# edwindn/rl-agent-for-qubit-array-tuning

Measured on AMD Instinct MI355X. Metric: env steps/sec (batched 8-dot 64x64 CSD solves), higher is better.
Workload: dtype f64; 1 GPU; 8-dot array, 4096 parallel envs per GPU, 64x64 CSD, deterministic physics (latching/noise off), 50-step episodes, staggered phases: 820 episode resets (new device + first observation) inside the timed region, synthetic CNN outputs; n_dots=8, envs_per_gpu=4096, resolution=64

## Files before the change

### __graft_entry__.py

```python
import os
import subprocess
import sys

ROOT = os.path.dirname(os.path.abspath(__file__))
PKG = os.path.join(ROOT, "rl-agent-for-qubit-array-tuning_amd")
for _p in (PKG, os.path.join(ROOT, "oracle"), os.path.join(ROOT, "tests")):
    if _p not in sys.path:
        sys.path.insert(0, _p)


def build() -> None:
    csrc = os.path.join(PKG, "csrc")
    subprocess.check_call(["make", "-C", csrc, "libqdsim.so"])
    subprocess.check_call(["make", "-C", os.path.join(ROOT, "tests", "hosttest"), "libqdsim_hosttest.so", "qd_scratch_asan"])
    subprocess.check_call(["make", "-C", os.path.join(ROOT, "tests", "hosttest_wave"), "libqdsim_hosttest_wave.so"])
    subprocess.check_call(["make", "-C", os.path.join(ROOT, "tests", "hosttest_gs"), "libqdsim_hosttest_gs.so"])
    subprocess.check_call(["make", "-C", os.path.join(ROOT, "tests", "hosttest_points"), "libqdsim_hosttest_points.so"])
    subprocess.check_call(["make", "-C", os.path.join(ROOT, "tests", "hosttest_latch"), "libqdsim_hosttest_latch.so"])
    subprocess.check_call(["make", "-C", os.path.join(ROOT, "tests", "gputest_eig"), "libqdsim_gputest_eig.so"])
    subprocess.check_call(["make", "-C", os.path.join(ROOT, "oracle"), "libqdoracle.so"])
    import qadapt_hip
    from qadapt_hip import _lib
    L = _lib.lib()
    missing = [n for n in _lib.EXPORTS if not hasattr(L, n)]
    if missing:
        raise RuntimeError(f"libqdsim.so lacks symbols: {missing}")


def smoke() -> None:
    import numpy as np
    import torch
    import qd_oracle as O
    import helpers as H
    from qadapt_hip.vec_env import VecQuantumDeviceEnv, SyntheticCapacitanceModel

    assert torch.cuda.is_available(), "smoke() needs the MI355X"
    N, R, B, seed = 4, 16, 2, 2024
    env = VecQuantumDeviceEnv(B, num_dots=N, resolution=R, seed=seed, validate=True,
                              capacitance_model=SyntheticCapacitanceModel(3))
    rng = np.random.default_rng(0)
    C = N - 1
    v0 = rng.normal(0, 0.1, (B, C, 3)).astype(np.float32); l0 = rng.uniform(-6, -2, (B, C, 3)).astype(np.float32)
    obs = env.reset(cnn_outputs=(torch.as_tensor(v0).cuda(), torch.as_tensor(l0).cuda()))
    act = rng.uniform(-1, 1, (B, 2 * N - 1)).astype(np.float32)
    v1 = rng.normal(0, 0.1, (B, C, 3)).astype(np.float32); l1 = rng.uniform(-6, -2, (B, C, 3)).astype(np.float32)
    obs, rew, term, trunc = env.step(torch.as_tensor(act).cuda(),
                                     cnn_outputs=(torch.as_tensor(v1).cuda(), torch.as_tensor(l1).cuda()))
    img = obs["image"].cpu().numpy()
    raw, _ = env.raw()
    for e in range(B):
        oe = O.OracleEnv(N, R)
        oe.reset(O.sample_episode(np.random.default_rng(seed + e), N), v0[e], l0[e])
        oobs, (gr, br), _, _ = oe.step(act[e, :N], act[e, N:], v1[e], l1[e])
        r = rew[e].cpu().numpy()
        assert np.allclose(r[:N], gr, rtol=1e-9) and np.allclose(r[N:], br, rtol=1e-9), "reward mismatch"
        H.image_parity(oe, img[e], raw[e])
    env.close()
    print("smoke ok: 4-dot 16x16 batched step matches the oracle")


if __name__ == "__main__":
    build()
    if len(sys.argv) > 1 and sys.argv[1] == "smoke":
        smoke()
```

### include/qdsim.h

```cpp
#ifndef QDSIM_H
#define QDSIM_H

#include <stdint.h>

#ifdef __cplusplus
extern "C" {
#endif

#define QD_OK 0
#define QD_ERR_ARG 1
#define QD_ERR_HIP 2
#define QD_ERR_STATE 3
#define QD_ERR_NOMEM 4

#define QD_FLAG_VALIDATE 1
#define QD_FLAG_PIXEL_SEARCH 2
#define QD_FLAG_RETIRED_TILE_FUSED 4

#define QD_NOISE_SENSOR 1
#define QD_NOISE_RADIAL 2
#define QD_NOISE_LATCH 4

typedef struct qd_handle qd_handle;

typedef struct qd_config {
    int32_t struct_size;
    int32_t n_dot;
    int32_t resolution;
    int32_t batch;
    int32_t max_steps;
    int32_t env_chunk;
    int32_t flags;
    int32_t noise_flags;
    double gate_ramp_start;
    double gate_quadratic_start;
    double barrier_ramp_start;
    double kalman_prior_mean;
    double kalman_prior_variance;
    double kalman_prior_mean_nnn;
    double kalman_variance_threshold;
    double kalman_process_noise;
    uint64_t rng_seed;
    int64_t env_id_offset;
    int32_t use_deltas;
    int32_t sparse_reward;
    int32_t gate_curve_type;
    int32_t update_method;
    int32_t cnn_outputs;
    int32_t num_charge_states;
    double delta_max;
    double gate_curve_exponent;
    double plunger_radius;
    double outer_plunger_radius;
    double outer_plunger_reward_max;
    double barrier_radius;
} qd_config;

#define QD_ALL_CHARGE_STATES(m) (-(m))

#define QD_CURVE_CONSTANT 0
#define QD_CURVE_POLYNOMIAL 1
#define QD_CURVE_EXPONENTIAL 2
#define QD_CURVE_LINEAR 3
#define QD_UPDATE_KALMAN 0
#define QD_UPDATE_DIRECT 1

int qd_param_block_doubles(int n_dot);
int qd_state_block_doubles(int n_dot);
int qd_layout_query(int n_dot, int32_t* out31);

// ... 75 lines not shown
```

### rl-agent-for-qubit-array-tuning_amd/csrc/qd_api.hip

```cpp
#include <hip/hip_runtime.h>
#include <stdio.h>
#include <stdlib.h>
#include <string.h>
#include <new>

#include "qdsim.h"
#include "qd_kernels.h"
#include "qd_fullspace.h"
#include "qd_probe.h"
#include "qd_latch.h"
#include "qd_points.h"
#include "qd_scratch.h"

struct QdStream : QdNoCopy {
    hipStream_t s = nullptr;
    ~QdStream() { if (s) (void)hipStreamDestroy(s); }
    hipError_t create() { return hipStreamCreateWithFlags(&s, hipStreamNonBlocking); }
};
struct QdEvent : QdNoCopy {
    hipEvent_t e = nullptr;
    ~QdEvent() { if (e) (void)hipEventDestroy(e); }
    hipError_t create(unsigned flags = hipEventDisableTiming) { return hipEventCreateWithFlags(&e, flags); }
};

// ... 409 lines not shown
    nz.env_off = b.env_off;
    nz.ser_lo = (uint32_t)b.serial; nz.ser_hi = (uint32_t)(b.serial >> 32);
    nz.tel = b.tel; nz.tel_words = b.tel_words;
    return nz;
}

enum {
    QD_ST_TILE = 1, QD_ST_REDO = 2, QD_ST_STRUCTURE = 4, QD_ST_SOLVE = 8, QD_ST_SELECT = 16,
    QD_ST_SEARCH = QD_ST_TILE | QD_ST_REDO,
    QD_ST_GROUND = QD_ST_STRUCTURE | QD_ST_SOLVE | QD_ST_SELECT,
    QD_ST_ALL = QD_ST_SEARCH | QD_ST_GROUND
};

static int qd_stages(const qd_handle* h) {
    return h->full_m ? QD_ST_GROUND : (h->tile_search ? QD_ST_ALL : QD_ST_ALL & ~QD_ST_TILE);
}

template <int BIN>
static hipError_t qd_launch_solve(const qd_handle* h, const QdLane& ln, hipStream_t s) {
    const dim3 grid((unsigned)h->solve_grid[BIN]);
    QD_DISPATCH_BOOL(qd_validate(h), VAL,
                     qd_k_gs_solve<BIN, VAL><<<grid, dim3(256), 0, s>>>(ln.slabs.p, ln.gtiles.p, ln.gtiles.p + 16, h->gs_batches, h->tstats.p));
    return hipGetLastError();
}

static int qd_launch_ground(const qd_handle* h, const QdEnvBufs& b, const QdLane& ln, const int32_t* env_ids, int base, int cnt,
                            hipStream_t s, int st) {
    const int nb = (h->P + h->ppb - 1) / h->ppb;
    unsigned* tilelist = ln.gtiles.p + 16;
    const bool val = qd_validate(h);
    QdWide wide = h->wide; wide.buf = ln.wide.p;
    const int rec0 = val ? base : 0;
    for (int off = 0; off < cnt; off += h->gs_chunk) {
        const int n = cnt - off < h->gs_chunk ? cnt - off : h->gs_chunk;
        const QdGsGeom g{n, h->C, h->P, nb};
        const unsigned batches = (unsigned)((size_t)n * h->C * nb);
        if (st & QD_ST_STRUCTURE) {
            QD_HIP(hipMemsetAsync(ln.gtiles.p, 0, sizeof(unsigned) * 16, s));
            if (h->full_m) {
#define QD_DISPATCH_FULL(...)                                                                                  \
                if (!wide.capw && h->full_spl == 2) { constexpr int SPL = 2; constexpr bool WIDE = false; __VA_ARGS__; }  \
                else if (h->full_spl == 2) { constexpr int SPL = 2; constexpr bool WIDE = true; __VA_ARGS__; }            \
                else if (h->full_spl == 4) { constexpr int SPL = 4; constexpr bool WIDE = true; __VA_ARGS__; }            \
                else { constexpr int SPL = 8; constexpr bool WIDE = true; __VA_ARGS__; }
                QD_DISPATCH_BOOL(val, VAL, QD_DISPATCH_FULL(QD_DISPATCH_N(h->N,
                    qd_k_full_structure<NN, VAL, SPL, WIDE><<<dim3(batches), dim3(64 * QdFullWpb<SPL>::v), 0, s>>>(env_ids, base + off,
                        rec0 + off, g, h->ppb, h->R, b.params, b.state, b.noise_flags, h->ftab.p, ln.recs.p, ln.slabs.p, ln.gtiles.p, tilelist,
                        h->gs_batches, wide))));
#undef QD_DISPATCH_FULL
            } else {
                QD_DISPATCH_BOOL(val, VAL, QD_DISPATCH_BOOL(batches < (unsigned)h->cus, SMALL, QD_DISPATCH_N(h->N,
                    qd_k_gs_structure<NN, VAL, (SMALL ? 16 : 4)><<<dim3(batches), dim3(64 * (SMALL ? 16 : 4)), 0, s>>>(env_ids, base + off,
                        rec0 + off, g, h->R, b.params, ln.recs.p, b.state, b.noise_flags, ln.slabs.p, ln.gtiles.p, tilelist, h->gs_batches,
                        h->kept))));
            }
            QD_HIP(hipGetLastError());
        }
        if (st & QD_ST_SOLVE) {
            int max_bin = h->N == 2 ? qd_gs_bin(4) : (h->N == 3 ? qd_gs_bin(12) : QD_GS_NBIN - 1);
            if (h->full_m) {
                int M = 0, maxsec = 0;
                qd_full_sizes(h->N, h->full_m, M, maxsec);
                max_bin = qd_gs_bin(maxsec < QD_K ? maxsec : QD_K);
            } else if (h->kept < 2) max_bin = -1;
            else if (qd_gs_bin(h->kept) < max_bin) max_bin = qd_gs_bin(h->kept);
            const bool forked = max_bin >= 9;
            hipStream_t s9 = forked ? ln.side.s : s, s48 = forked ? ln.side2.s : s;
            if (forked) {
                QD_HIP(hipEventRecord(ln.ev_fork.e, s));
                QD_HIP(hipStreamWaitEvent(ln.side.s, ln.ev_fork.e, 0));
                QD_HIP(hipStreamWaitEvent(ln.side2.s, ln.ev_fork.e, 0));
            }
            if (wide.capw) {
                const size_t slots = (size_t)batches * wide.capw, full = (size_t)h->cus * 4;
                const dim3 wgrid((unsigned)(slots < full ? slots : full));
                QD_DISPATCH_BOOL(val, VAL, qd_k_full_solve_wide<VAL><<<wgrid, dim3(64), 0, s>>>(ln.slabs.p, wide, batches, h->tstats.p));
                QD_HIP(hipGetLastError());
            }
            if (max_bin >= 9) QD_HIP(qd_launch_solve<9>(h, ln, s9));
            if (forked) QD_HIP(hipEventRecord(ln.ev_join.e, ln.side.s));
            if (max_bin >= 8) QD_HIP(qd_launch_solve<8>(h, ln, s48));
            if (max_bin >= 7) QD_HIP(qd_launch_solve<7>(h, ln, s48));
            if (max_bin >= 6) QD_HIP(qd_launch_solve<6>(h, ln, s48));
            if (max_bin >= 5) QD_HIP(qd_launch_solve<5>(h, ln, s48));
            if (max_bin >= 4) QD_HIP(qd_launch_solve<4>(h, ln, s48));
            if (forked) QD_HIP(hipEventRecord(ln.ev_join2.e, ln.side2.s));
            if (max_bin >= 0) QD_HIP(qd_launch_solve<0>(h, ln, s));
            if (max_bin >= 1) QD_HIP(qd_launch_solve<1>(h, ln, s));
            if (max_bin >= 2) QD_HIP(qd_launch_solve<2>(h, ln, s));
            if (max_bin >= 3) QD_HIP(qd_launch_solve<3>(h, ln, s));
            if (forked) {
                QD_HIP(hipStreamWaitEvent(s, ln.ev_join.e, 0));
                QD_HIP(hipStreamWaitEvent(s, ln.ev_join2.e, 0));
            }
        }
        if (st & QD_ST_SELECT) {
            if (h->full_m) {
                const unsigned blk = (unsigned)((h->ppb + 63) / 64 * 64);
                QD_DISPATCH_BOOL(val, VAL, QD_DISPATCH_BOOL(wide.capw != 0, WIDE, QD_DISPATCH_N(h->N,
                    qd_k_full_select<NN, VAL, WIDE><<<dim3(batches), dim3(blk), 0, s>>>(env_ids, base + off, rec0 + off, g, h->ppb,
                        b.params, ln.recs.p, b.zraw, b.occ, b.state, b.noise_flags, b.eig, h->ftab.p, ln.slabs.p, wide))));
            } else {
                QD_DISPATCH_BOOL(val, VAL, QD_DISPATCH_N(h->N, QD_DISPATCH_KC(h->kc,
                    qd_k_gs_select<NN, VAL, KK><<<dim3(batches), dim3(QD_GS_BLOCK), 0, s>>>(env_ids, base + off, rec0 + off, g, h->R,
                        b.params, ln.recs.p, b.zraw, b.occ, b.state, b.noise_flags, b.eig, ln.slabs.p))));
            }
            QD_HIP(hipGetLastError());
// ... 547 lines not shown
```

### rl-agent-for-qubit-array-tuning_amd/csrc/qd_groundstate.h

```cpp
#pragma once
#include "qd_pixel.h"
#include "qd_eig.h"

#define QD_GS_PPB 256
#define QD_GS_NBIN 10
QD_HD constexpr int qd_gs_bin(int s) { return s <= 8 ? s - 2 : (s <= 10 ? 7 : (s <= 12 ? 8 : 9)); }
QD_HD constexpr int qd_gs_bin_min(int bin) { return bin <= 6 ? bin + 2 : (bin == 7 ? 9 : (bin == 8 ? 11 : 13)); }

QD_HD unsigned qd_gs_hop(unsigned ci, unsigned cj, unsigned tcq) {
#if defined(__HIP_DEVICE_COMPILE__)
    unsigned ay;
    asm("v_sad_u32 %0, %1, %2, 0" : "=v"(ay) : "v"(ci), "v"(cj));
#else
    const unsigned ay = ci > cj ? ci - cj : cj - ci;
#endif
    const int tz = __builtin_ctz(ay | 0x80000000u);
    const unsigned x = ay + (0xFFFFFFF1u << tz);
    const unsigned t = (tcq >> tz) & 1u;
    return t > x ? t - x : 0u;
}

#if defined(__HIPCC__)

#ifndef QD_NBREG
#define QD_NBREG 6
#endif
#define QD_GS_BLOCK 256
#define QD_LINK_NONE 0xFFFFFFFFu
#define QD_LINK_SINGLE 0xFFFFFFFEu

typedef __attribute__((address_space(3))) double qd_lds_double;
typedef volatile qd_lds_double* qd_lds_vptr;
typedef const volatile qd_lds_double* qd_lds_cvptr;

template <int N>
struct QdWaveLds {
    static constexpr int NS = (2 * (N - 1) - QD_NBREG) > 1 ? (2 * (N - 1) - QD_NBREG) : 1;
    double coef[NS][64];
    unsigned char nidx[NS][64];
    double buf[64];
    double pv[2][16];
    short pfl[2][8];
};
struct QdBlockLds {
    unsigned pool_top;
    unsigned cnt[QD_GS_NBIN];
};

struct QdSlab {
    double* pool; unsigned* link; unsigned char* rank; unsigned* lists; double* aux; unsigned* cnt; double* lam;
};
constexpr int QD_GS_CAP_TAB[QD_GS_NBIN + 1] = {16, 10, 8, 6, 5, 4, 4, 3, 2, 2, 2};
constexpr int QD_GS_OFF_TAB[QD_GS_NBIN + 1] = {0, 16, 26, 34, 40, 45, 49, 53, 56, 58, 60};
constexpr unsigned long long qd_gs_pack_tab(const int* tab, int n, int bits) {
    unsigned long long w = 0;
    for (int b = 0; b < n; ++b) w |= (unsigned long long)tab[b] << (bits * b);
    return w;
}
constexpr unsigned long long QD_GS_CAP_WORD = qd_gs_pack_tab(QD_GS_CAP_TAB, QD_GS_NBIN + 1, 5);
constexpr unsigned long long QD_GS_OFF_WORD = qd_gs_pack_tab(QD_GS_OFF_TAB, QD_GS_NBIN, 6);
QD_HD constexpr int qd_gs_list_cap(int bin) { return QD_GS_PPB * (int)((QD_GS_CAP_WORD >> (5 * bin)) & 31u); }
QD_HD constexpr int qd_gs_list_off(int bin) {
    return QD_GS_PPB * (bin >= QD_GS_NBIN ? QD_GS_OFF_TAB[QD_GS_NBIN] : (int)((QD_GS_OFF_WORD >> (6 * bin)) & 63u));
}
constexpr bool qd_gs_lists_match_definition() {
    int o = 0;
    for (int b = 0; b <= QD_GS_NBIN; ++b) {
        if (qd_gs_list_off(b) != o || qd_gs_list_cap(b) != QD_GS_PPB * (32 / qd_gs_bin_min(b))) return false;
        o += QD_GS_PPB * (32 / qd_gs_bin_min(b));
    }
    return true;
}
static_assert(qd_gs_lists_match_definition(), "QD_GS_CAP_TAB / QD_GS_OFF_TAB: capacity 32 / qd_gs_bin_min(b) per pixel, offsets their running sum");
__host__ __device__ inline int qd_gs_task_doubles(int s, bool validate) {
    const int ne = s * (s + 1) / 2;
    const int n = 2 + ne + (s > QD_EIG_REG ? 4 * s + (validate ? ne : 0) : 0);
    return (n + 1) & ~1;
}
__host__ __device__ inline size_t qd_gs_pool_doubles(bool validate) { return (size_t)QD_GS_PPB * (size_t)qd_gs_task_doubles(32, validate); }
__host__ __device__ inline size_t qd_gs_slab_bytes(bool validate) {
    size_t b = qd_gs_pool_doubles(validate) * 8;
    b += (size_t)QD_GS_PPB * 32 * 4;
    b += (size_t)qd_gs_list_off(QD_GS_NBIN) * 4;
    b += (size_t)QD_GS_PPB * 16;
    b += (size_t)QD_GS_PPB * 32;
    b += 64;
    b += (size_t)qd_gs_list_off(QD_GS_NBIN) * 8;
    return (b + 255) & ~(size_t)255;
}
__host__ __device__ inline QdSlab qd_gs_slab(unsigned char* base, bool validate) {
    QdSlab s;
    s.pool = (double*)base; base += qd_gs_pool_doubles(validate) * 8;
    s.link = (unsigned*)base; base += (size_t)QD_GS_PPB * 32 * 4;
    s.lists = (unsigned*)base; base += (size_t)qd_gs_list_off(QD_GS_NBIN) * 4;
    s.aux = (double*)base; base += (size_t)QD_GS_PPB * 16;
    s.rank = base; base += (size_t)QD_GS_PPB * 32;
    s.cnt = (unsigned*)base; base += 64;
    s.lam = (double*)base;
    return s;
}
__host__ __device__ inline size_t qd_gs_tile_cap(int bin, size_t batches) { return batches * (size_t)((qd_gs_list_cap(bin) + 63) / 64); }
__host__ __device__ inline size_t qd_gs_tile_off(int bin, size_t batches) { size_t o = 0; for (int b = 0; b < bin; ++b) o += qd_gs_tile_cap(b, batches); return o; }

__device__ __forceinline__ unsigned qd_half_ballot(bool p) {
    unsigned long long b = __ballot(p);
    return (unsigned)(b >> (threadIdx.x & 32));
}
__device__ __forceinline__ double qd_half_min(double v) {
#pragma unroll
    for (int o = 16; o > 0; o >>= 1) v = fmin(v, __shfl_xor(v, o, 32));
    return v;
}
__device__ __forceinline__ int qd_wave_max_int(int v) {
#pragma unroll
    for (int o = 32; o > 0; o >>= 1) v = max(v, __shfl_xor(v, o, 64));
    return __builtin_amdgcn_readfirstlane(v);
}

#ifndef QD_GS_ROT_SWIZZLE
#define QD_GS_ROT_SWIZZLE 1
#endif
template <int J, bool UP>
__device__ __forceinline__ unsigned qd_half_rot(unsigned v) {
#if QD_GS_ROT_SWIZZLE
    return (unsigned)__builtin_amdgcn_ds_swizzle((int)v, 0xC000 | ((UP ? 0 : 1) << 10) | (J << 5));
#else
    return (unsigned)__shfl((int)v, ((int)(threadIdx.x & 31) + (UP ? J : 32 - J)) & 31, 32);
#endif
}
template <int J>
__device__ __forceinline__ void qd_gs_hop_rounds(unsigned ecode, unsigned tcq, unsigned& acc) {
    const unsigned hop = qd_gs_hop(ecode, qd_half_rot<J, true>(ecode), tcq);
    acc |= hop << J;
    if constexpr (J < 16) {
        acc |= qd_half_rot<J, false>(hop) << (32 - J);
        qd_gs_hop_rounds<J + 1>(ecode, tcq, acc);
    }
}

template <int N, bool VALIDATE>
__device__ __forceinline__ void qd_ground_structure(const QdPixelRec* __restrict__ rec, bool live, int ps, QdWaveLds<N>& W,
                                                    QdBlockLds& S, const QdSlab& sl, int kept) {
    const int lane = threadIdx.x & 63;
    const int m = lane & 31;
    const int hb = lane & 32;
    const unsigned lt = (1u << m) - 1u;
    qd_lds_vptr buf = (qd_lds_vptr)W.buf;

    const int hh = hb >> 5;
    if (m >= 9 && m < 9 + N - 1) W.pv[hh][m] = rec->tc[m - 9];
    if (m >= 16 && m < 16 + N) W.pfl[hh][m - 16] = (short)rec->fl[m - 16];
    __builtin_amdgcn_wave_barrier();
    const double* pvv = W.pv[hh];
    const bool inK = m < kept;
    const int nvalid = min(rec->nvalid, kept);
    const bool valid = m < nvalid;
    const unsigned code = valid ? (unsigned)rec->idx[m] : 0u;
    unsigned ecode = code;
    ecode = (ecode | (ecode << 8)) & 0x00FF00FFu;
    ecode = (ecode | (ecode << 4)) & 0x0F0F0F0Fu;
    ecode = (ecode | (ecode << 2)) & 0x33333333u;
    const double Fabs = inK ? rec->E[m] : INFINITY;
    const double fshift = qd_half_min(Fabs);
    const double F = Fabs - fshift;

    unsigned tcnz = 0;
#pragma unroll
    for (int d = 0; d < N - 1; ++d) tcnz |= (pvv[9 + d] != 0.0 ? 1u : 0u) << d;
    unsigned tcq = 0;
#pragma unroll
    for (int q = 0; q < N - 1; ++q) tcq |= ((tcnz >> (N - 2 - q)) & 1u) << (4 * q);
    unsigned acc = 0;
    qd_gs_hop_rounds<1>(ecode, tcq, acc);
    unsigned nbrmask = __builtin_rotateleft32(acc, (unsigned)m);
    nbrmask = (valid && live) ? (nbrmask & (nvalid >= 32 ? 0xFFFFFFFFu : ((1u << nvalid) - 1u))) : 0u;
#if defined(QD_ABLATE) && QD_ABLATE == 4
    nbrmask = 0;
#endif
    const int cnt = __popc(nbrmask);
    const int maxcnt = qd_wave_max_int(cnt);
    double radius = 0.0;
    double creg[QD_NBREG]; int jreg[QD_NBREG];
#pragma unroll
    for (int i = 0; i < QD_NBREG; ++i) { creg[i] = 0.0; jreg[i] = m; }
    {
        unsigned rem = nbrmask;
        for (int s = 0; s < maxcnt; ++s) {
            const bool has = rem != 0;
            const int j = has ? __builtin_ctz(rem) : m;
            rem &= rem - 1;
            const unsigned cj = __shfl(ecode, j, 32);
            double c = 0.0;
            if (has) {
                const int Y = (int)cj - (int)ecode;
                const unsigned ay = (unsigned)(Y < 0 ? -Y : Y);
                const int q = __builtin_ctz(ay) >> 2;
                const int d = N - 2 - q;
                const int nd = (int)W.pfl[hh][d] + (int)((ecode >> (4 * (q + 1))) & 3u) - 1;
                const int nd1 = (int)W.pfl[hh][d + 1] + (int)((ecode >> (4 * q)) & 3u) - 1;
                const double t = pvv[9 + d];
                const double prod = (double)((Y < 0) ? nd * (nd1 + 1) : nd1 * (nd + 1));
                double sq_ = 0.0;
                if (prod > 0.0) sq_ = qd_sqrt1(prod);
                c = -t * sq_;
            }
            if (s < QD_NBREG) {
#pragma unroll
                for (int i = 0; i < QD_NBREG; ++i) if (i == s) { creg[i] = c; jreg[i] = j; }
            } else { W.coef[s - QD_NBREG][lane] = c; W.nidx[s - QD_NBREG][lane] = (unsigned char)j; }
            radius += fabs(c);
        }
    }

    unsigned seg = (1u << m) | nbrmask;
    for (int guard = 0; guard < 32; ++guard) {
        unsigned nw = seg, rem = nbrmask;
        for (int s = 0; s < maxcnt; ++s) {
            const bool has = rem != 0;
            const int j = has ? __builtin_ctz(rem) : m;
            rem &= rem - 1;
            nw |= __shfl(seg, j, 32);
        }
        const bool changed = nw != seg;
        seg = nw;
        if (!__any(changed)) break;
    }
    const int ssz = __popc(seg);
    const int r = __popc(seg & lt);
    const int smax = qd_wave_max_int(ssz);

    double comp_lower;
    {
        buf[lane] = F - radius;
        __builtin_amdgcn_wave_barrier();
        double acc = INFINITY;
        unsigned mm = seg;
        for (int it = 0; it < smax; ++it) {
            if (mm) { const int b = __builtin_ctz(mm); mm &= mm - 1; acc = fmin(acc, buf[hb + b]); }
        }
        __builtin_amdgcn_wave_barrier();
        comp_lower = acc;
    }
    const bool active = live && comp_lower <= 0.0;
#if defined(QD_ABLATE) && QD_ABLATE == 3
    const bool solve = false;
#else
    const bool solve = active && ssz > 1;
#endif

    unsigned base = 0, gi = 0;
    if (solve && r == 0) {
        base = atomicAdd(&S.pool_top, (unsigned)qd_gs_task_doubles(ssz, VALIDATE));
        const int bin = qd_gs_bin(ssz);
        gi = (unsigned)qd_gs_list_off(bin) + atomicAdd(&S.cnt[bin], 1u);
        sl.lists[gi] = base;
        if (ssz > 8) sl.pool[base + 1] = (double)ssz;
    }
    base = (unsigned)__shfl((int)base, __builtin_ctz(seg), 32);
    gi = (unsigned)__shfl((int)gi, __builtin_ctz(seg), 32);
    if (live) {
        sl.link[ps * 32 + m] = solve ? gi : (active ? QD_LINK_SINGLE : QD_LINK_NONE);
        sl.rank[ps * 32 + m] = (unsigned char)r;
        if (VALIDATE) {
            const double hn = -qd_half_min(inK ? -(fabs(Fabs) + radius) : INFINITY);
            if (m == 0) { sl.aux[ps] = hn; sl.aux[QD_GS_PPB + ps] = fshift; }
        }
    }
    {
        double* row = sl.pool + base + 2 + (r * (r + 1)) / 2;
        unsigned nrm = 0;
        for (int s = 0; s < maxcnt; ++s) {
            if (s < cnt && solve) {
                int j = jreg[0]; double c = creg[0];
                if (s >= QD_NBREG) { j = (int)W.nidx[s - QD_NBREG][lane]; c = W.coef[s - QD_NBREG][lane]; }
#pragma unroll
                for (int i = 1; i < QD_NBREG; ++i) if (i == s) { j = jreg[i]; c = creg[i]; }
                const int rj = __popc(seg & ((1u << j) - 1u));
                if (rj < r) { row[rj] = c; nrm |= 1u << rj; }
            }
        }
        for (int c = 0; c < smax - 1; ++c)
            if (solve && c < r && !((nrm >> c) & 1u)) row[c] = 0.0;
        if (solve) row[r] = F;
    }
}

template <int S, bool PADDED, bool VALIDATE>
__device__ __forceinline__ int qd_eig_task(double* rec, double& lam) {
    double resid, x[S];
    int its = 0;
    const int sz = PADDED ? (int)rec[1] : S;
    qd_eig_lowest<S, VALIDATE>(rec + 2, lam, x, resid, VALIDATE ? &its : nullptr, sz);
    if (VALIDATE) rec[1] = resid;
    if (sz == S) {
        double2* X2 = reinterpret_cast<double2*>(rec + 2);
#pragma unroll
        for (int i = 0; i + 1 < S; i += 2) X2[i >> 1] = make_double2(x[i], x[i + 1]);
        if (S & 1) rec[2 + S - 1] = x[S - 1];
    } else {
#pragma unroll
        for (int i = 0; i < S; ++i) if (i < sz) rec[2 + i] = x[i];
    }
    return its;
}
template <bool VALIDATE>
__device__ __forceinline__ int qd_eig_task_mem(double* rec, double& lam) {
    const int s = (int)rec[1];
    const int ne = s * (s + 1) / 2;
    double* M = rec + 2;
    double* work = M + ne;
    double* copy = VALIDATE ? work + 4 * s : nullptr;
    if (VALIDATE) for (int e = 0; e < ne; ++e) copy[e] = M[e];
    double resid;
    int its = 0;
    qd_eig_lowest_mem(s, M, work, copy, lam, resid, VALIDATE ? &its : nullptr);
    if (VALIDATE) rec[1] = resid;
    for (int i = 0; i < s; ++i) M[i] = work[3 * s + i];
    return its;
}

template <int N, bool VALIDATE, int KC>
__device__ __forceinline__ void qd_ground_select(const QdPixelRec* __restrict__ rec, int ps, const QdSlab& sl,
                                                 double* occ, double& lam_out, double& resid_out) {
    const unsigned* __restrict__ link = sl.link + ps * 32;
    const unsigned char* __restrict__ rank = sl.rank + ps * 32;
    const double* __restrict__ pool = sl.pool;
    const double* __restrict__ lamd = sl.lam;
    const int nvalid = rec->nvalid;
    unsigned lk[KC];
    double lam[KC];
    {
        const uint4* l4 = reinterpret_cast<const uint4*>(link);
#pragma unroll
        for (int q = 0; q < KC / 4; ++q) { const uint4 v = l4[q]; lk[4 * q] = v.x; lk[4 * q + 1] = v.y; lk[4 * q + 2] = v.z; lk[4 * q + 3] = v.w; }
// ... 64 lines not shown
```

### rl-agent-for-qubit-array-tuning_amd/csrc/qd_kernels.h

```cpp
#pragma once
#include "qd_groundstate.h"
#include "qd_rng.h"

#if defined(__HIPCC__)

struct QdRewardCfg {
    double gate_ramp_start, gate_quadratic_start, barrier_ramp_start;
    int max_steps;
    int use_deltas, sparse, curve;
    double delta_max, curve_exponent;
    double plunger_radius, outer_plunger_radius, outer_plunger_reward_max, barrier_radius;
};

__device__ __forceinline__ double qd_gate_reward(double dist, const QdRewardCfg& rc) {
    if (rc.sparse) {
        if (dist <= rc.plunger_radius) return 1.0;
        if (dist <= rc.outer_plunger_radius) {
            const double nd = (dist - rc.plunger_radius) / (rc.outer_plunger_radius - rc.plunger_radius);
            return rc.outer_plunger_reward_max * (1.0 - nd);
        }
        return 0.0;
    }
    double r;
    if (dist >= rc.gate_ramp_start) r = 0.0;
// ... 163 lines not shown
    if (nv < KC) {
        double dd[N];
#pragma unroll
        for (int i = 0; i < N; ++i) dd[i] = 0.0 - vd[i];
#pragma unroll 1
        for (int i = 0; i < N; ++i) {
            const double t = qd_dotN<N>(spar + L.cdd_inv + i * G, dd);
            double di = dd[0];
#pragma unroll
            for (int j = 1; j < N; ++j) di = (j == i) ? dd[j] : di;
            F0 = fma(di, t, F0);
        }
    }
#pragma unroll
    for (int m = 0; m < KC; ++m) rec->E[m] = (m < nv ? se[m * QD_CAND_BLOCK + threadIdx.x] : F0) * isa;
#pragma unroll
    for (int i = 0; i < N; ++i) rec->fl[i] = fl[i];
    rec->nvalid = nv;
}

struct QdGsGeom { int n_env, C, P, nb; };
__device__ __forceinline__ void qd_gs_locate(const QdGsGeom& g, int batch, int& slot, int& ch, int& p0) {
    slot = batch / (g.C * g.nb);
    const int rem = batch - slot * g.C * g.nb;
    ch = rem / g.nb; p0 = (rem - ch * g.nb) * QD_GS_PPB;
}

__device__ __forceinline__ void qd_gs_publish_tiles(const QdBlockLds& sB, const QdSlab& sl, int batch, unsigned* __restrict__ gtiles,
                                                    unsigned* __restrict__ tilelist, size_t batches_cap) {
    if (threadIdx.x < QD_GS_NBIN) {
        const int bin = threadIdx.x;
        const unsigned nt = sB.cnt[bin];
        sl.cnt[bin] = nt;
        const unsigned ntile = (nt + 63u) >> 6;
        if (ntile) {
            const unsigned start = atomicAdd(&gtiles[bin], ntile);
            unsigned* tl = tilelist + qd_gs_tile_off(bin, batches_cap) + start;
            for (unsigned t = 0; t < ntile; ++t) {
                const unsigned here = nt - t * 64u < 64u ? nt - t * 64u : 64u;
                tl[t] = ((unsigned)batch << 12) | (t << 6) | (here - 1u);
            }
        }
    }
}

#ifndef QD_GS_WAVES
#define QD_GS_WAVES 7
#endif
template <int N, bool VALIDATE, int WPB>
__global__ void __launch_bounds__(64 * WPB, WPB == 4 ? QD_GS_WAVES : 4)
qd_k_gs_structure(const int* __restrict__ env_ids, int env_base, int rec_slot0, QdGsGeom g, int R, const double* __restrict__ params,
                  const QdPixelRec* __restrict__ recs, const double* __restrict__ state, int noise_flags,
                  unsigned char* __restrict__ slabs, unsigned* __restrict__ gtiles, unsigned* __restrict__ tilelist, size_t batches_cap,
                  int kept) {
    const QdLayout L = qd_layout(N);
    __shared__ QdWaveLds<N> sW[WPB];
    __shared__ QdBlockLds sB;
    constexpr int PPW = QD_GS_PPB / WPB;
    const int batch = blockIdx.x;
    const QdSlab sl = qd_gs_slab(slabs + (size_t)batch * qd_gs_slab_bytes(VALIDATE), VALIDATE);
    const int wave = threadIdx.x >> 6, lane = threadIdx.x & 63;
    int slot, ch, p0;
    qd_gs_locate(g, batch, slot, ch, p0);
    const int e = env_ids ? env_ids[env_base + slot] : env_base + slot;
    const double* par = params + (size_t)e * L.size;
    const double* st = state + (size_t)e * L.s_size;
    if (qd_radial_replaced(par, st, L, ch, noise_flags)) {
        if (threadIdx.x < QD_GS_NBIN) sl.cnt[threadIdx.x] = 0;
        return;
    }
    const QdPixelRec* rbase = recs + ((size_t)(rec_slot0 + slot) * g.C + ch) * g.P;
    if (threadIdx.x <= QD_GS_NBIN) { if (threadIdx.x == 0) sB.pool_top = 0; else sB.cnt[threadIdx.x - 1] = 0; }
    __syncthreads();
    QdWaveLds<N>& W = sW[wave];
    for (int it = 0; it < PPW / 2; ++it) {
        const int ps = wave * PPW + it * 2 + (lane >> 5);
        if (p0 + wave * PPW + it * 2 >= g.P) break;
        const int p = p0 + ps;
        const int pc = p < g.P ? p : g.P - 1;
        qd_ground_structure<N, VALIDATE>(rbase + pc, p < g.P, ps, W, sB, sl, kept);
    }
    __syncthreads();
    qd_gs_publish_tiles(sB, sl, batch, gtiles, tilelist, batches_cap);
}

template <int BIN, bool VALIDATE>
__device__ __forceinline__ int qd_gs_solve_task(double* rec, double& lam) {
    if constexpr (BIN <= 6) return qd_eig_task<BIN + 2, false, VALIDATE>(rec, lam);
    else if constexpr (BIN == 7) return qd_eig_task<10, true, VALIDATE>(rec, lam);
    else if constexpr (BIN == 8) return qd_eig_task<12, true, VALIDATE>(rec, lam);
    else return qd_eig_task_mem<VALIDATE>(rec, lam);
}
template <int BIN> struct QdGsSolveWaves { static constexpr int v = BIN <= 1 ? 6 : (BIN == 2 ? 4 : (BIN == 3 ? 3 : (BIN <= 6 ? 2 : (BIN == 9 ? 4 : 1)))); };

template <int BIN, bool VALIDATE>
__global__ void __launch_bounds__(256, QdGsSolveWaves<BIN>::v)
qd_k_gs_solve(unsigned char* __restrict__ slabs, const unsigned* __restrict__ gtiles, const unsigned* __restrict__ tilelist,
              size_t batches_cap, unsigned long long* __restrict__ stats) {
    const int lane = threadIdx.x & 63;
    const unsigned ntile = gtiles[BIN];
    const unsigned* tl = tilelist + qd_gs_tile_off(BIN, batches_cap);
    const unsigned nwaves = gridDim.x * 4u;
    unsigned gt = blockIdx.x * 4u + (threadIdx.x >> 6);
    const size_t slab_bytes = qd_gs_slab_bytes(VALIDATE);
    auto offset_of = [&](unsigned d) -> unsigned {
        const QdSlab sl = qd_gs_slab(slabs + (size_t)(d >> 12) * slab_bytes, VALIDATE);
        return lane <= (int)(d & 63u) ? sl.lists[qd_gs_list_off(BIN) + (int)((d >> 6) & 63u) * 64 + lane] : 0u;
    };
    unsigned desc = gt < ntile ? tl[gt] : 0u;
    unsigned desc1 = gt + nwaves < ntile ? tl[gt + nwaves] : 0u;
    unsigned off = gt < ntile ? offset_of(desc) : 0u;
    for (; gt < ntile; gt += nwaves) {
        const unsigned desc2 = gt + 2u * nwaves < ntile ? tl[gt + 2u * nwaves] : 0u;
        const unsigned off1 = gt + nwaves < ntile ? offset_of(desc1) : 0u;
        const unsigned batch = desc >> 12;
        const int here = (int)(desc & 63u) + 1;
        const QdSlab sl = qd_gs_slab(slabs + (size_t)batch * slab_bytes, VALIDATE);
        int its = 0;
        if (lane < here) {
            double lam;
            its = qd_gs_solve_task<BIN, VALIDATE>(sl.pool + off, lam);
            sl.lam[qd_gs_list_off(BIN) + (int)((desc >> 6) & 63u) * 64 + lane] = lam;
        }
        desc = desc1; desc1 = desc2; off = off1;
        if (VALIDATE && stats) {
            int sum = its, mx = its;
#pragma unroll
            for (int o = 32; o > 0; o >>= 1) { sum += __shfl_xor(sum, o, 64); mx = max(mx, __shfl_xor(mx, o, 64)); }
            if (lane == 0) {
                atomicAdd(&stats[16], (unsigned long long)here); atomicAdd(&stats[17], (unsigned long long)sum);
                atomicAdd(&stats[18], 1ull); atomicAdd(&stats[19], (unsigned long long)mx);
                atomicAdd(&stats[20 + BIN], (unsigned long long)here);
            }
// ... 579 lines not shown
```

### rl-agent-for-qubit-array-tuning_amd/qadapt_hip/_lib.py

```python
from __future__ import annotations

import ctypes
import os
import subprocess

_HERE = os.path.dirname(os.path.abspath(__file__))
CSRC = os.path.join(os.path.dirname(_HERE), "csrc")
LIB_PATH = os.environ.get("QDSIM_LIB", os.path.join(CSRC, "libqdsim.so"))

QD_FLAG_VALIDATE = 1
QD_FLAG_PIXEL_SEARCH = 2
QD_NOISE_SENSOR = 1
QD_NOISE_RADIAL = 2
QD_NOISE_LATCH = 4
QD_MAP_GLOBAL, QD_MAP_PER_SCAN = 0, 1
QD_POINTS_SLOTS = 64
QD_ERR_ARG, QD_ERR_HIP, QD_ERR_STATE = 1, 2, 3

EXPORTS = [
    "qd_param_block_doubles", "qd_state_block_doubles", "qd_layout_query", "qd_create", "qd_destroy",
    "qd_last_error", "qd_bind_outputs", "qd_load_episodes", "qd_apply_actions", "qd_observe",
    "qd_update_capacitance", "qd_step", "qd_snapshot", "qd_get_state", "qd_set_state", "qd_get_raw",
    "qd_get_occupations", "qd_get_candidates", "qd_get_eigen", "qd_get_search_stats", "qd_get_solver_stats", "qd_get_rng_state", "qd_set_rng_state",
    "qd_time_ground_kernel", "qd_time_candidates_kernel", "qd_time_kernels", "qd_timed_kernel_name", "qd_chunk_envs",
    "qd_probe", "qd_probe_compose", "qd_time_select", "qd_eval_points", "qd_probe_ex",
]

QD_CURVES = {"constant": 0, "polynomial": 1, "exponential": 2, "linear": 3}
QD_UPDATE_KALMAN, QD_UPDATE_DIRECT = 0, 1


class QdConfig(ctypes.Structure):
    _fields_ = [
        ("struct_size", ctypes.c_int32), ("n_dot", ctypes.c_int32), ("resolution", ctypes.c_int32),
        ("batch", ctypes.c_int32), ("max_steps", ctypes.c_int32), ("env_chunk", ctypes.c_int32),
        ("flags", ctypes.c_int32), ("noise_flags", ctypes.c_int32),
        ("gate_ramp_start", ctypes.c_double), ("gate_quadratic_start", ctypes.c_double),
        ("barrier_ramp_start", ctypes.c_double), ("kalman_prior_mean", ctypes.c_double),
        ("kalman_prior_variance", ctypes.c_double), ("kalman_prior_mean_nnn", ctypes.c_double),
        ("kalman_variance_threshold", ctypes.c_double), ("kalman_process_noise", ctypes.c_double),
        ("rng_seed", ctypes.c_uint64), ("env_id_offset", ctypes.c_int64),
        ("use_deltas", ctypes.c_int32), ("sparse_reward", ctypes.c_int32), ("gate_curve_type", ctypes.c_int32),
        ("update_method", ctypes.c_int32), ("cnn_outputs", ctypes.c_int32), ("num_charge_states", ctypes.c_int32),
        ("delta_max", ctypes.c_double), ("gate_curve_exponent", ctypes.c_double),
        ("plunger_radius", ctypes.c_double), ("outer_plunger_radius", ctypes.c_double),
        ("outer_plunger_reward_max", ctypes.c_double), ("barrier_radius", ctypes.c_double),
    ]


class QdProbeOpts(ctypes.Structure):
    _fields_ = [
        ("struct_size", ctypes.c_int32), ("noise_flags", ctypes.c_int32), ("serial", ctypes.c_uint64),
        ("stream_base", ctypes.c_int64), ("occ_dst", ctypes.c_void_p),
    ]


class QdError(RuntimeError):
    pass


def build(force=False):
    if force and os.path.exists(LIB_PATH):
        os.remove(LIB_PATH)
    subprocess.check_call(["make", "-s", "-C", CSRC, "libqdsim.so"])
# ... 72 lines not shown
```

### rl-agent-for-qubit-array-tuning_amd/qadapt_hip/vec_env.py

```python
from __future__ import annotations

import ctypes

import numpy as np
import torch

from . import _lib
from .device_model import DeviceSampler, check_solver_options, load_yaml, max_charge_carriers
from .layout import layout


class SyntheticCapacitanceModel:

    def __init__(self, seed=99, outputs=3):
        self.seed = seed
        self.calls = 0
        self.outputs = outputs

    def __call__(self, images):
        n = images.shape[0]
        g = torch.Generator(device="cpu").manual_seed(self.seed + self.calls)
        self.calls += 1
        values = torch.randn((n, self.outputs), generator=g, dtype=torch.float32) * 0.1
        log_vars = torch.rand((n, self.outputs), generator=g, dtype=torch.float32) * 4.0 - 6.0
# ... 9 lines not shown
            "current_barrier_voltages": st[:, L.s_barrier_v:L.s_barrier_v + N - 1].copy(),
            "virtual_gate_matrix": st[:, L.s_vgm:L.s_vgm + G * G].reshape(-1, G, G).copy(),
            "virtual_gate_origin": params[:, L.origin:L.origin + G].copy(),
            "kalman_means": st[:, L.s_kmean:L.s_kmean + N * N].reshape(-1, N, N).copy(),
            "kalman_variances": st[:, L.s_kvar:L.s_kvar + N * N].reshape(-1, N, N).copy(),
            "steps": steps}


def cgd_full_from_params(L, params):
    return params[:, L.cgd:L.cgd + L.G * L.V].reshape(-1, L.G, L.V).copy()


def override_charge_states(qconfig, num_charge_states):
    if num_charge_states is not None:
        qconfig["simulator"].setdefault("latched_model", {})["num_charge_states"] = \
            None if num_charge_states == "all" else num_charge_states
    return qconfig


def make_qd_config(config, qconfig, num_dots, resolution, batch, *, env_chunk=0, flags=0, noise_flags=0, seed=0,
                   env_id_offset=0):
    sim, rew, cm = config["simulator"], config["reward"], config["capacitance_model"]
    nearest = bool(cm.get("nearest_neighbour"))
    k = check_solver_options(qconfig, n_dot=num_dots)
    ncs = k if k is not None else -max_charge_carriers(qconfig)
    return _lib.QdConfig(struct_size=ctypes.sizeof(_lib.QdConfig), n_dot=int(num_dots), resolution=int(resolution),
                         batch=int(batch), max_steps=int(sim["max_steps"]), env_chunk=int(env_chunk), flags=int(flags),
                         noise_flags=int(noise_flags),
                         gate_ramp_start=float(rew["gate_ramp_start"]),
                         gate_quadratic_start=float(rew["gate_quadratic_start"]),
                         barrier_ramp_start=float(rew["barrier_ramp_start"]),
                         kalman_prior_mean=0.3, kalman_prior_variance=0.5, kalman_prior_mean_nnn=0.15,
                         kalman_variance_threshold=float(cm.get("variance_threshold", 0.05)),
                         kalman_process_noise=float(cm.get("process_noise", 0.0)),
                         rng_seed=int(seed) & 0xFFFFFFFFFFFFFFFF, env_id_offset=int(env_id_offset),
                         use_deltas=1 if sim.get("use_deltas") else 0,
                         sparse_reward=1 if rew.get("sparse_reward") else 0,
                         gate_curve_type=_lib.QD_CURVES[rew.get("gate_curve_type", "constant")],
                         update_method=_lib.QD_UPDATE_DIRECT if cm["update_method"] == "direct" else _lib.QD_UPDATE_KALMAN,
                         cnn_outputs=2 if nearest else 3, num_charge_states=ncs,
                         delta_max=float(sim.get("delta_max", 0.0)),
                         gate_curve_exponent=float(rew.get("gate_curve_exponent", 2.0)),
                         plunger_radius=float(rew.get("plunger_radius", 0.0)),
                         outer_plunger_radius=float(rew.get("outer_plunger_radius", 0.0)),
                         outer_plunger_reward_max=float(rew.get("outer_plunger_reward_max", 0.0)),
                         barrier_radius=float(rew.get("barrier_radius", 0.0)))


class VecQuantumDeviceEnv:
    def __init__(self, num_envs, num_dots=None, config_path=None, qarray_config_path=None,
                 resolution=None, device=None, seed=None, env_id_offset=0, capacitance_model=None,
                 validate=False, env_chunk=0, reset_kalman_on_reset=False, noise=None,
                 vary_peak_width=False, peak_width_alpha=0.01, voltage_capacitance_model=None, pixel_search=False,
                 num_charge_states=None):
        if seed is None:
            seed = int(np.random.SeedSequence().entropy) & 0x7FFFFFFFFFFF
        self.seed = int(seed)
        self.env_id_offset = int(env_id_offset)
        self.config = load_yaml(config_path, "env_config.yaml")
        self.qconfig = load_yaml(qarray_config_path, "qarray_config.yaml")
        override_charge_states(self.qconfig, num_charge_states)
        if voltage_capacitance_model is not None:
            self.qconfig["simulator"]["voltage_capacitance_model"]["type"] = \
                None if voltage_capacitance_model in ("none", "null") else voltage_capacitance_model
        sim = self.config["simulator"]
        self.num_envs = int(num_envs)
        self.num_dots = int(num_dots if num_dots is not None else sim["num_dots"])
        self.num_charge_states = check_solver_options(self.qconfig, n_dot=self.num_dots)
        self.max_charge_carriers = max_charge_carriers(self.qconfig) if self.num_charge_states is None else None
        self.use_barriers = bool(sim["use_barriers"])
        if not self.use_barriers:
            raise NotImplementedError("env.py only supports barrier mode for now")
        rew = self.config["reward"]
        if rew.get("gate_curve_type", "constant") not in _lib.QD_CURVES:
            raise ValueError(f"Unknown curve type: {rew.get('gate_curve_type')}")
        self.resolution = int(resolution if resolution is not None else sim["resolution"])
        self.max_steps = int(sim["max_steps"])
        self.update_method = self.config["capacitance_model"]["update_method"]
        if self.update_method in ("bayesian", "kriging", "ema"):
            raise NotImplementedError(f"update_method={self.update_method!r} requires an updater module the "
                                      "reference removed; use 'kalman' or 'direct'")
        if self.update_method == "fake":
            raise ValueError("update_method 'fake' fails in the reference's barrier mode (shape mismatch in "
                             "QarrayBaseClass._update_virtual_gate_matrix); not built")
        if self.update_method not in (None, "kalman", "direct", "perfect"):
            raise ValueError(f"Unknown update method: {self.update_method}")
        self.nearest_neighbour = bool(self.config["capacitance_model"].get("nearest_neighbour"))
        self.cnn_outputs = 2 if self.nearest_neighbour else 3
        if self.update_method in (None, "perfect"):
            capacitance_model = None
        self.capacitance_model = capacitance_model
        if self.update_method in ("kalman", "direct") and capacitance_model is None:
            raise RuntimeError("Error initialising capacitance model: update_method 'kalman' needs a "
                               "capacitance_model callable (images -> values, log_vars)")
        if not torch.cuda.is_available():
            raise RuntimeError("VecQuantumDeviceEnv needs a ROCm GPU (no CPU fallback)")
        self.device = torch.device(device if device is not None else "cuda")
        if self.device.index is None:
            self.device = torch.device("cuda", torch.cuda.current_device())
        self.reset_kalman_on_reset = bool(reset_kalman_on_reset)
        N = self.num_dots; R = self.resolution; B = self.num_envs
        self.N, self.R, self.B, self.C = N, R, B, N - 1
        self.L = layout(N)
        self.sampler = DeviceSampler(N, self.qconfig, self.config, vary_peak_width=vary_peak_width,
                                     peak_width_alpha=peak_width_alpha,
                                     perfect_vgm=self.update_method == "perfect")
        self._rngs = [np.random.Generator(np.random.PCG64(self.seed + self.env_id_offset + e)) for e in range(B)]
        self._lib = _lib.lib()
        self.noise_flags = self._noise_flags(noise)
        self._probe_serials = 0
        cfg = make_qd_config(self.config, self.qconfig, N, R, B, env_chunk=env_chunk,
                             flags=(_lib.QD_FLAG_VALIDATE if validate else 0) | (_lib.QD_FLAG_PIXEL_SEARCH if pixel_search else 0),
                             noise_flags=self.noise_flags, seed=self.seed, env_id_offset=self.env_id_offset)
        self._h = ctypes.c_void_p()
        rc = self._lib.qd_create(ctypes.byref(cfg), self.device.index, ctypes.byref(self._h))
        if rc != 0:
            msg = self._lib.qd_last_error(self._h).decode() if self._h else "no handle"
            if self._h:
                self._lib.qd_destroy(self._h)
                self._h = None
            raise _lib.QdError(f"qd_create failed (code {rc}): {msg}")
        self.validate = bool(validate)
        dev = self.device
        self.global_image = torch.zeros((B, R, R, self.C), dtype=torch.float32, device=dev)
        self.plunger_images = torch.zeros((B, N, R, R, 2), dtype=torch.float32, device=dev)
        self.barrier_images = torch.zeros((B, self.C, R, R, 1), dtype=torch.float32, device=dev)
        self.voltages = torch.zeros((B, 2 * N - 1), dtype=torch.float32, device=dev)
        self.rewards = torch.zeros((B, 2 * N - 1), dtype=torch.float64, device=dev)
        self.truncated = torch.zeros((B,), dtype=torch.uint8, device=dev)
        _lib.check(self._h, self._lib.qd_bind_outputs(self._h, self.global_image.data_ptr(),
                                                      self.plunger_images.data_ptr(),
                                                      self.barrier_images.data_ptr(),
                                                      self.voltages.data_ptr()), "qd_bind_outputs")
        self._params_host = np.zeros((B, self.L.size))
        self._steps_host = np.zeros(B, np.int64)
        self._needs_reset = True
        self.obs_count = 0
        self.final = None

    def _noise_flags(self, noise):
        if not noise:
            return 0
        if noise is True:
            rn = self.config["simulator"].get("radial_noise") or {}
            lt = self.qconfig["simulator"]["model"].get("latching_model_parameters") or {}
            return (_lib.QD_NOISE_SENSOR | (_lib.QD_NOISE_RADIAL if rn.get("enabled") else 0)
                    | (_lib.QD_NOISE_LATCH if lt.get("Exists") else 0))
        f = 0
        for k in noise:
            f |= {"sensor": _lib.QD_NOISE_SENSOR, "radial": _lib.QD_NOISE_RADIAL, "latch": _lib.QD_NOISE_LATCH}[k]
        return f

    def _stream(self):
        return ctypes.c_void_p(torch.cuda.current_stream(self.device).cuda_stream)

    def close(self):
        if getattr(self, "_h", None) is not None and self._h:
            self._lib.qd_destroy(self._h)
            self._h = None

    def __del__(self):
        try:
            self.close()
        except Exception:
            pass
# ... 358 lines not shown
```

Before: 13030 env-steps/s.

## Prune ground-state solves with a pairwise upper bound instead of the Gershgorin zero test

Computes a per-half-wave upper bound on the minimum energy from pairwise 2x2 bounds, plus a norm-scaled margin. A component is solved only if its Gershgorin lower bound falls below that bound, rather than whenever it is at or below zero. This is meant to skip more small eigen-solves in the ground-state structure kernel. The change also adds a DPP-based f64 half-wave min reduction, packs neighbour indices into one register, and bounds the row-zeroing loop by the largest solved segment. The old zero criterion stays available behind a new flag. The extra LDS write, reduction and wave barriers add cost, and the bound must never prune a true ground state.

Measured after the change: 13260 env-steps/s, median of 6. +1.7%, better.

```diff
diff --git a/__graft_entry__.py b/__graft_entry__.py
--- a/__graft_entry__.py
+++ b/__graft_entry__.py
@@ -15,6 +15,7 @@
     subprocess.check_call(["make", "-C", os.path.join(ROOT, "tests", "hosttest"), "libqdsim_hosttest.so", "qd_scratch_asan"])
     subprocess.check_call(["make", "-C", os.path.join(ROOT, "tests", "hosttest_wave"), "libqdsim_hosttest_wave.so"])
     subprocess.check_call(["make", "-C", os.path.join(ROOT, "tests", "hosttest_gs"), "libqdsim_hosttest_gs.so"])
+    subprocess.check_call(["make", "-C", os.path.join(ROOT, "tests", "hosttest_prune"), "libqdsim_hosttest_prune.so"])
     subprocess.check_call(["make", "-C", os.path.join(ROOT, "tests", "hosttest_points"), "libqdsim_hosttest_points.so"])
     subprocess.check_call(["make", "-C", os.path.join(ROOT, "tests", "hosttest_latch"), "libqdsim_hosttest_latch.so"])
     subprocess.check_call(["make", "-C", os.path.join(ROOT, "tests", "gputest_eig"), "libqdsim_gputest_eig.so"])
diff --git a/include/qdsim.h b/include/qdsim.h
--- a/include/qdsim.h
+++ b/include/qdsim.h
@@ -16,6 +16,7 @@
 #define QD_FLAG_VALIDATE 1
 #define QD_FLAG_PIXEL_SEARCH 2
 #define QD_FLAG_RETIRED_TILE_FUSED 4
+#define QD_FLAG_GS_GERSHGORIN_ZERO 8
 
 #define QD_NOISE_SENSOR 1
 #define QD_NOISE_RADIAL 2
diff --git a/rl-agent-for-qubit-array-tuning_amd/csrc/qd_api.hip b/rl-agent-for-qubit-array-tuning_amd/csrc/qd_api.hip
--- a/rl-agent-for-qubit-array-tuning_amd/csrc/qd_api.hip
+++ b/rl-agent-for-qubit-array-tuning_amd/csrc/qd_api.hip
@@ -485,7 +485,7 @@
                 QD_DISPATCH_BOOL(val, VAL, QD_DISPATCH_BOOL(batches < (unsigned)h->cus, SMALL, QD_DISPATCH_N(h->N,
                     qd_k_gs_structure<NN, VAL, (SMALL ? 16 : 4)><<<dim3(batches), dim3(64 * (SMALL ? 16 : 4)), 0, s>>>(env_ids, base + off,
                         rec0 + off, g, h->R, b.params, ln.recs.p, b.state, b.noise_flags, ln.slabs.p, ln.gtiles.p, tilelist, h->gs_batches,
-                        h->kept))));
+                        h->kept, (h->cfg.flags & QD_FLAG_GS_GERSHGORIN_ZERO) ? 1 : 0))));
             }
             QD_HIP(hipGetLastError());
         }
diff --git a/rl-agent-for-qubit-array-tuning_amd/csrc/qd_groundstate.h b/rl-agent-for-qubit-array-tuning_amd/csrc/qd_groundstate.h
--- a/rl-agent-for-qubit-array-tuning_amd/csrc/qd_groundstate.h
+++ b/rl-agent-for-qubit-array-tuning_amd/csrc/qd_groundstate.h
@@ -19,6 +19,10 @@
     const unsigned t = (tcq >> tz) & 1u;
     return t > x ? t - x : 0u;
 }
+
+QD_HD double qd_gs_pair_bound(double Fi, double Fj, double c) { return __builtin_fma(0.5, Fi + Fj, -__builtin_fabs(c)); }
+QD_HD double qd_gs_prune_margin(double hnorm) { return 0x1p-40 * hnorm; }
+QD_HD bool qd_gs_is_task(double comp_lower, double ub, double margin) { return comp_lower <= ub + margin; }
 
 #if defined(__HIPCC__)
 
@@ -106,10 +110,27 @@
     unsigned long long b = __ballot(p);
     return (unsigned)(b >> (threadIdx.x & 32));
 }
+#ifndef QD_GS_MIN_DPP
+#define QD_GS_MIN_DPP 1
+#endif
+template <int CTRL>
+__device__ __forceinline__ double qd_dpp_f64(double v) {
+    const int lo = __double2loint(v), hi = __double2hiint(v);
+    return __hiloint2double(__builtin_amdgcn_update_dpp(hi, hi, CTRL, 0xF, 0xF, false),
+                            __builtin_amdgcn_update_dpp(lo, lo, CTRL, 0xF, 0xF, false));
+}
 __device__ __forceinline__ double qd_half_min(double v) {
+#if QD_GS_MIN_DPP
+    v = fmin(v, qd_dpp_f64<0xB1>(v));
+    v = fmin(v, qd_dpp_f64<0x4E>(v));
+    v = fmin(v, qd_dpp_f64<0x141>(v));
+    v = fmin(v, qd_dpp_f64<0x140>(v));
+    return fmin(v, __shfl_xor(v, 16, 32));
+#else
 #pragma unroll
     for (int o = 16; o > 0; o >>= 1) v = fmin(v, __shfl_xor(v, o, 32));
     return v;
+#endif
 }
 __device__ __forceinline__ int qd_wave_max_int(int v) {
 #pragma unroll
@@ -140,7 +161,7 @@
 
 template <int N, bool VALIDATE>
 __device__ __forceinline__ void qd_ground_structure(const QdPixelRec* __restrict__ rec, bool live, int ps, QdWaveLds<N>& W,
-                                                    QdBlockLds& S, const QdSlab& sl, int kept) {
+                                                    QdBlockLds& S, const QdSlab& sl, int kept, bool bound0) {
     const int lane = threadIdx.x & 63;
     const int m = lane & 31;
     const int hb = lane & 32;
@@ -180,10 +201,15 @@
     const int cnt = __popc(nbrmask);
     const int maxcnt = qd_wave_max_int(cnt);
     double radius = 0.0;
-    double creg[QD_NBREG]; int jreg[QD_NBREG];
-#pragma unroll
-    for (int i = 0; i < QD_NBREG; ++i) { creg[i] = 0.0; jreg[i] = m; }
-    {
+    double ubl = 0.0;
+    double creg[QD_NBREG];
+    unsigned jpack = 0;
+    static_assert(5 * QD_NBREG <= 32, "jpack: 5 bits per register slot");
+#pragma unroll
+    for (int i = 0; i < QD_NBREG; ++i) creg[i] = 0.0;
+    {
+        buf[lane] = F;
+        __builtin_amdgcn_wave_barrier();
         unsigned rem = nbrmask;
         for (int s = 0; s < maxcnt; ++s) {
             const bool has = rem != 0;
@@ -203,12 +229,19 @@
                 double sq_ = 0.0;
                 if (prod > 0.0) sq_ = qd_sqrt1(prod);
                 c = -t * sq_;
+                ubl = fmin(ubl, qd_gs_pair_bound(F, buf[hb + j], c));
             }
             if (s < QD_NBREG) {
 #pragma unroll
-                for (int i = 0; i < QD_NBREG; ++i) if (i == s) { creg[i] = c; jreg[i] = j; }
+                for (int i = 0; i < QD_NBREG; ++i) if (i == s) creg[i] = c;
+                jpack |= (unsigned)j << (5 * s);
             } else { W.coef[s - QD_NBREG][lane] = c; W.nidx[s - QD_NBREG][lane] = (unsigned char)j; }
             radius += fabs(c);
+        }
+        if (!bound0) {
+            const double ub = qd_half_min(ubl);
+            const double hnorm = -qd_half_min(inK ? -(F + radius) : 0.0);
+            if (m == 0) { W.pv[hh][0] = ub; W.pv[hh][1] = qd_gs_prune_margin(hnorm); }
         }
     }
 
@@ -231,6 +264,7 @@
 
     double comp_lower;
     {
+        __builtin_amdgcn_wave_barrier();
         buf[lane] = F - radius;
         __builtin_amdgcn_wave_barrier();
         double acc = INFINITY;
@@ -241,12 +275,14 @@
         __builtin_amdgcn_wave_barrier();
         comp_lower = acc;
     }
-    const bool active = live && comp_lower <= 0.0;
+    bool active = live && comp_lower <= 0.0;
+    if (!bound0 && ssz > 1) active = live && qd_gs_is_task(comp_lower, pvv[0], pvv[1]);
 #if defined(QD_ABLATE) && QD_ABLATE == 3
     const bool solve = false;
 #else
     const bool solve = active && ssz > 1;
 #endif
+    const int smax_solve = qd_wave_max_int(solve ? ssz : 0);
 
     unsigned base = 0, gi = 0;
     if (solve && r == 0) {
@@ -271,15 +307,16 @@
         unsigned nrm = 0;
         for (int s = 0; s < maxcnt; ++s) {
             if (s < cnt && solve) {
-                int j = jreg[0]; double c = creg[0];
+                int j; double c = creg[0];
                 if (s >= QD_NBREG) { j = (int)W.nidx[s - QD_NBREG][lane]; c = W.coef[s - QD_NBREG][lane]; }
-#pragma unroll
-                for (int i = 1; i < QD_NBREG; ++i) if (i == s) { j = jreg[i]; c = creg[i]; }
+                else j = (int)((jpack >> (5 * s)) & 31u);
+#pragma unroll
+                for (int i = 1; i < QD_NBREG; ++i) if (i == s) c = creg[i];
                 const int rj = __popc(seg & ((1u << j) - 1u));
                 if (rj < r) { row[rj] = c; nrm |= 1u << rj; }
             }
         }
-        for (int c = 0; c < smax - 1; ++c)
+        for (int c = 0; c < smax_solve - 1; ++c)
             if (solve && c < r && !((nrm >> c) & 1u)) row[c] = 0.0;
         if (solve) row[r] = F;
     }
diff --git a/rl-agent-for-qubit-array-tuning_amd/csrc/qd_kernels.h b/rl-agent-for-qubit-array-tuning_amd/csrc/qd_kernels.h
--- a/rl-agent-for-qubit-array-tuning_amd/csrc/qd_kernels.h
+++ b/rl-agent-for-qubit-array-tuning_amd/csrc/qd_kernels.h
@@ -239,7 +239,7 @@
 qd_k_gs_structure(const int* __restrict__ env_ids, int env_base, int rec_slot0, QdGsGeom g, int R, const double* __restrict__ params,
                   const QdPixelRec* __restrict__ recs, const double* __restrict__ state, int noise_flags,
                   unsigned char* __restrict__ slabs, unsigned* __restrict__ gtiles, unsigned* __restrict__ tilelist, size_t batches_cap,
-                  int kept) {
+                  int kept, int bound0) {
     const QdLayout L = qd_layout(N);
     __shared__ QdWaveLds<N> sW[WPB];
     __shared__ QdBlockLds sB;
@@ -265,7 +265,7 @@
         if (p0 + wave * PPW + it * 2 >= g.P) break;
         const int p = p0 + ps;
         const int pc = p < g.P ? p : g.P - 1;
-        qd_ground_structure<N, VALIDATE>(rbase + pc, p < g.P, ps, W, sB, sl, kept);
+        qd_ground_structure<N, VALIDATE>(rbase + pc, p < g.P, ps, W, sB, sl, kept, bound0 != 0);
     }
     __syncthreads();
     qd_gs_publish_tiles(sB, sl, batch, gtiles, tilelist, batches_cap);
diff --git a/rl-agent-for-qubit-array-tuning_amd/qadapt_hip/_lib.py b/rl-agent-for-qubit-array-tuning_amd/qadapt_hip/_lib.py
--- a/rl-agent-for-qubit-array-tuning_amd/qadapt_hip/_lib.py
+++ b/rl-agent-for-qubit-array-tuning_amd/qadapt_hip/_lib.py
@@ -10,6 +10,7 @@
 
 QD_FLAG_VALIDATE = 1
 QD_FLAG_PIXEL_SEARCH = 2
+QD_FLAG_GS_GERSHGORIN_ZERO = 8
 QD_NOISE_SENSOR = 1
 QD_NOISE_RADIAL = 2
 QD_NOISE_LATCH = 4
diff --git a/rl-agent-for-qubit-array-tuning_amd/qadapt_hip/vec_env.py b/rl-agent-for-qubit-array-tuning_amd/qadapt_hip/vec_env.py
--- a/rl-agent-for-qubit-array-tuning_amd/qadapt_hip/vec_env.py
+++ b/rl-agent-for-qubit-array-tuning_amd/qadapt_hip/vec_env.py
@@ -85,7 +85,7 @@
                  resolution=None, device=None, seed=None, env_id_offset=0, capacitance_model=None,
                  validate=False, env_chunk=0, reset_kalman_on_reset=False, noise=None,
                  vary_peak_width=False, peak_width_alpha=0.01, voltage_capacitance_model=None, pixel_search=False,
-                 num_charge_states=None):
+                 num_charge_states=None, gs_gershgorin_zero=False):
         if seed is None:
             seed = int(np.random.SeedSequence().entropy) & 0x7FFFFFFFFFFF
         self.seed = int(seed)
@@ -143,7 +143,8 @@
         self.noise_flags = self._noise_flags(noise)
         self._probe_serials = 0
         cfg = make_qd_config(self.config, self.qconfig, N, R, B, env_chunk=env_chunk,
-                             flags=(_lib.QD_FLAG_VALIDATE if validate else 0) | (_lib.QD_FLAG_PIXEL_SEARCH if pixel_search else 0),
+                             flags=(_lib.QD_FLAG_VALIDATE if validate else 0) | (_lib.QD_FLAG_PIXEL_SEARCH if pixel_search else 0)
+                             | (_lib.QD_FLAG_GS_GERSHGORIN_ZERO if gs_gershgorin_zero else 0),
                              noise_flags=self.noise_flags, seed=self.seed, env_id_offset=self.env_id_offset)
         self._h = ctypes.c_void_p()
         rc = self._lib.qd_create(ctypes.byref(cfg), self.device.index, ctypes.byref(self._h))
```
